# mdw771/beyond_dof

Hardware: AMD Instinct MI355X
Metric: multislice fwd+adjoint slice-steps/s (full Adam iteration: rotation, forward, loss, adjoint, gradient exchange, regulariser+Adam) (higher is better)
Workload: dtype f32

## Files before the change

### beyond_dof_amd/csrc/bdof_capi.hip

```cpp
#include <hip/hip_runtime.h>
#include <hip/hip_ext.h>
#include <cmath>
#include <algorithm>
#include <complex>
#include <cstdio>
#include <cstdlib>
#include <cstring>
#include <string>
#include <vector>

#include "../../include/bdof.h"
#include "bdof_steps.h"
#include "bdof_kernels.h"
#include "bdof_conv2.h"
#include "bdof_generic.h"
#include "bdof_field.h"
#include "bdof_conv64.h"
#include "bdof_resident.h"
#include "bdof_modes.h"
#include "bdof_comm.h"
#include "bdof_rigid.h"
#include "bdof_windows.h"
#include <rocfft/rocfft.h>
#include <map>
// ... 631 lines not shown
                    tw_of(c, c->twX, c->NX, tick)};
    sq_of(c, tick, a.sq);
    DISPATCH_N(c->NX, {
        if (gather) BDOF_LAUNCH(ps, (k_row_prop_gather<N_>), dim3(rows_grid<N_>(c, g.B, c->NY)), dim3(BDOF_THREADS), 0, g.st, a);
        else BDOF_LAUNCH(ps, (k_row_prop_fan<N_>), dim3(rows_grid<N_>(c, g.B, c->NY)), dim3(BDOF_THREADS), 0, g.st, a);
    });
}

static int fused_mode(const bdof_ctx* c) {
    if (c->fusion < 1 || c->sep_copies < 1 || c->recompute || c->bin != 1 || c->pstack || c->range_car) return 0;
    if (c->det_mode == BDOF_DET_FAR || c->obj.xoff || c->obj.yoff || c->gpsi0) return 0;
    if (c->S < 4 || (c->S & 1) || c->NX > 512 || c->NY > 512) return 0;
    return 1;
}
static LineSteps line_steps(bdof_ctx* c, bool x_lines, unsigned lead, unsigned trail) {
    const int N = x_lines ? c->NX : c->NY;
    const cf* tw = x_lines ? c->twX : c->twY;
    const cf* h = x_lines ? c->hx_d : c->hy_d;
    const unsigned D = (unsigned)c->sep_copies;
    LineSteps s{tw_of(c, tw, N, lead), tw_of(c, tw, N, trail), h + (size_t)(lead % D) * N, h + (size_t)(trail % D) * N};
    sq_of(c, lead, s.sq_lead);
    sq_of(c, trail, s.sq_trail);
    return s;
}
static void launch_slice(bdof_ctx* c, const Group& g, int z, const cf* in, cf* out, cf* phi, bool blk = false) {
    ProfScope ps(c, BDOF_K_ROW_FWD, g.st, true);
    const bool xl = (z & 1) != 0;
    const int N = xl ? c->NX : c->NY, R = xl ? c->NY : c->NX;
    SliceArgs a{sub_field(c, g, in), c->probe, sub_field(c, g, out), sub_field(c, g, phi), sub_obj(c, g), g.B, R, z, carrier_at(c, z), cshift_at(c, z),
                line_steps(c, xl, (unsigned)(z > 0 ? z - 1 : 0), (unsigned)z)};
    if (xl) {
        DISPATCH_N_512(N, with_bool(blk, [&](auto BLK) {
            BDOF_LAUNCH(ps, (k_slice_x<N_, BLK>), dim3(rows_grid<N_>(c, g.B, R)), dim3(BDOF_THREADS), 0, g.st, a);
        }));
    } else {
        DISPATCH_N_512(N, with_bool(z == 0, [&](auto FIRST) { with_bool(z == c->S - 2, [&](auto TAIL) {
            BDOF_LAUNCH(ps, (k_slice_y<N_, FIRST, TAIL>), dim3(rows_grid<N_>(c, g.B, R)), dim3(BDOF_THREADS), 0, g.st, a);
        }); }));
    }
}

static void launch_slice_adj(bdof_ctx* c, const Group& g, int z, const cf* in, cf* out, const cf* phi) {
    ProfScope ps(c, BDOF_K_ROW_BWD, g.st, true);
    const bool xl = (z & 1) != 0;
    const int N = xl ? c->NX : c->NY, R = xl ? c->NY : c->NX;
    SliceAdjArgs a{sub_field(c, g, in), sub_field(c, g, phi), sub_field(c, g, out), c->grot + (size_t)g.b0 * c->S * c->NX * c->NY, sub_obj(c, g), g.B, R, z,
                   c->k, carrier_phi_at(c, z), line_steps(c, xl, (unsigned)z, (unsigned)(z > 0 ? z - 1 : 0))};
    if (xl) {
        DISPATCH_N_512(N, BDOF_LAUNCH(ps, (k_slice_x_adj<N_>), dim3(rows_grid<N_>(c, g.B, R)), dim3(BDOF_THREADS), 0, g.st, a));
    } else {
        DISPATCH_N_512(N, with_bool(z == c->S - 2, [&](auto HEAD) { with_bool(z == 0, [&](auto LAST) {
            BDOF_LAUNCH(ps, (k_slice_y_adj<N_, HEAD, LAST>), dim3(rows_grid<N_>(c, g.B, R)), dim3(BDOF_THREADS), 0, g.st, a);
        }); }));
    }
}

struct GradTarget {
    float2* grot = nullptr;
    int S_ = 0, z_ = 0;
    cf* gpsi = nullptr;
};
static void launch_row_bwd(bdof_ctx* c, const Group& g, int z, const cf* gin, const cf* tape, cf* gout, int hist = 0, float tape_scale = 1.f,
                           const GradTarget* gt = nullptr) {
    ProfScope ps(c, BDOF_K_ROW_BWD, g.st, true);
    float2* grot = gt && gt->grot ? gt->grot + (size_t)g.b0 * gt->S_ * c->NX * c->NY : c->grot + (size_t)g.b0 * c->S * c->NX * c->NY;
    RowBwdArgs a{sub_field(c, g, gin), hist == 2 ? c->probe : sub_field(c, g, tape), sub_field(c, g, gout),
                 grot, sub_obj(c, g), g.B, c->NX, z, c->k, carrier_at(c, z), tw_of(c, c->twY, c->NY, (unsigned)z),
                 slice_carrier_field(c, z), adj_carrier_at(c, g, steps(c).steps_back(z)), cshift_at(c, z), carrier_phi_at(c, z), tape_scale,
                 gt && gt->gpsi ? sub_field(c, g, gt->gpsi) : (z == 0 ? sub_field<cf>(c, g, c->gpsi0) : nullptr),
                 gt && gt->grot ? gt->S_ : c->S, gt && gt->grot ? gt->z_ : steps(c).first_slice(z)};
    sq_of(c, (unsigned)z, a.sq);
    const int form = a.ac.gcar ? 2 : a.pz ? 1 : 0;
    if (c->bin > 1) {
        DISPATCH_N(c->NY, with_bool(hist == 2, [&](auto H2) { with_int<3>(form, [&](auto FORM) {
            BDOF_LAUNCH(ps, (k_row_bwd<N_, H2 ? 2 : 1, FORM == 1, FORM == 2, true>), dim3(rows_grid<N_>(c, g.B, c->NX)), dim3(BDOF_THREADS), 0, g.st, a);
        }); }));
        return;
    }
    DISPATCH_N(c->NY, with_int<4>(hist, [&](auto HIST) { with_int<3>(form, [&](auto FORM) {
        BDOF_LAUNCH(ps, (k_row_bwd<N_, HIST, FORM == 1, FORM == 2>), dim3(rows_grid<N_>(c, g.B, c->NX)), dim3(BDOF_THREADS), 0, g.st, a);
    }); }));
}

static LossArgs loss_args(bdof_ctx* c, const Group& g, const DetPlane& det, const cf* in, cf* out_hyb, cf* out_wave, const float* meas,
                          float in_scale, float out_scale, int part) {
    LossArgs a{};
    a.in = sub_field(c, g, in);
    a.out_hyb = sub_field(c, g, out_hyb);
    a.out_wave = sub_field(c, g, out_wave);
    a.meas = sub_field(c, g, meas);
    a.partial = c->partial + 2 * part;
    a.B = g.B;
    a.in_scale = in_scale;
    a.out_scale = out_scale;
    a.det = det;
    return a;
}
static int launch_loss_real(bdof_ctx* c, const Group& g, const DetPlane& det, const cf* in, cf* out_hyb, bool tstore, cf* out_wave, const float* meas,
                            float in_scale, float out_scale, int part = 0) {
    ProfScope ps(c, BDOF_K_LOSS, g.st);
    LossArgs a = loss_args(c, g, det, in, out_hyb, out_wave, meas, in_scale, out_scale, part);
    a.R = c->NX;
    a.twiddle = c->twY;
    int grid = 0;
    DISPATCH_N(c->NY, grid = rows_grid<N_>(c, g.B, c->NX); with_bool(tstore, [&](auto TSTORE) { with_bool(meas && loss_is_poisson(c), [&](auto PSN) {
        with_bool(meas && det.wgt, [&](auto WGT) { hipLaunchKernelGGL((k_row_loss<N_, false, TSTORE, PSN, WGT>), dim3(grid), dim3(BDOF_THREADS), 0, g.st, a); });
    }); }));
    return grid;
}

static int launch_loss_plane(bdof_ctx* c, const Group& g, const DetPlane& det, int j, cf* out_wave, const float* meas, int part = 0) {
    ProfScope ps(c, BDOF_K_LOSS, g.st);
    const size_t pl = (size_t)c->NX * c->NY;
    LossPlaneArgs a;
    static_cast<LossArgs&>(a) = loss_args(c, g, det, nullptr, nullptr, nullptr, nullptr, 1.f, 1.f, part);
    a.in = sub_planes<const cf>(c, g, c->det_pl) + j * pl;
    a.out_hyb = meas ? sub_planes<cf>(c, g, c->seed_pl) + j * pl : nullptr;
    a.out_wave = out_wave ? sub_planes(c, g, out_wave) + j * pl : nullptr;
    a.meas = meas ? sub_planes(c, g, meas) + j * pl : nullptr;
    a.fstride = c->planes;
    a.R = c->NX;
    a.twiddle = c->twY;
    int grid = 0;
    DISPATCH_N(c->NY, grid = rows_grid<N_>(c, g.B, c->NX); with_bool(meas && loss_is_poisson(c), [&](auto PSN) {
        with_bool(meas && det.wgt, [&](auto WGT) { hipLaunchKernelGGL((k_row_loss<N_, false, true, PSN, WGT, true>), dim3(grid), dim3(BDOF_THREADS), 0, g.st, a); });
    }));
    return grid;
}

static int launch_loss_far(bdof_ctx* c, const Group& g, const DetPlane& det, const cf* in, cf* out_hyb, cf* out_wave, const float* meas,
                           float in_scale, float out_scale, int part = 0) {
    ProfScope ps(c, BDOF_K_LOSS, g.st);
    LossArgs a = loss_args(c, g, det, in, out_hyb, out_wave, meas, in_scale, out_scale, part);
    a.R = c->NY;
    a.twiddle = c->twX;
    int grid = 0;
    DISPATCH_N(c->NX, grid = rows_grid<N_>(c, g.B, c->NY); with_bool(meas && loss_is_poisson(c), [&](auto PSN) {
        with_bool(meas && det.wgt, [&](auto WGT) { hipLaunchKernelGGL((k_row_loss<N_, true, true, PSN, WGT>), dim3(grid), dim3(BDOF_THREADS), 0, g.st, a); });
    }));
    return grid;
}

struct DetRoute {
    bool far;
    const cf* in;
    float in_scale;
    const cf* h;
    const cf* pfield;
};
static DetRoute det_route(const bdof_ctx* c) {
    const bool tf_all = c->variant == BDOF_VARIANT_TF_ALL;
    if (c->det_mode == BDOF_DET_FAR) return DetRoute{true, c->bufA, 1.f, nullptr, c->pdetT};
    if (c->det_mode == BDOF_DET_NONE && !tf_all) return DetRoute{false, c->bufA, 1.f / (float)c->NY, nullptr, c->pdet};
    return DetRoute{false, c->bufB, 1.f, c->det_mode == BDOF_DET_NONE ? c->hs : tf_all ? c->hcomb : c->hdet, c->pdet};
}

enum { TAPE_NONE = 0, TAPE_HISTORY = 1, TAPE_LAST = 2 };
static void forward_sweep(bdof_ctx* c, const Split& split, int tape_mode, bool fused = false, bool adj_fused = false) {
    const size_t fld = (size_t)c->Bmax * c->NX * c->NY;
    const DetRoute dr = det_route(c);
    const int nz = n_steps(c);
    for (int z = 0; z < nz; ++z) {
        const cf* in = nullptr;
        if (z > 0) in = tape_mode == TAPE_HISTORY ? c->tape + (size_t)steps(c).tape_read(z) * fld : c->bufB;
        const bool last = z == nz - 1;
        if (fused && last) in = c->tape + (size_t)z * fld;
        if (fused && !last) {
            for (const Group& g : split) {
                launch_slice(c, g, z, (z & 1) ? c->bufA : c->bufB, (z & 1) ? c->bufB : c->bufA, c->tape + (size_t)z * fld, adj_fused);
                if (z == nz - 2) launch_row_prop(c, g, c->bufA, c->tape + (size_t)(nz - 1) * fld, c->hx_rows, 1.f, 0, z, BDOF_K_LOSS);
            }
            continue;
        }
        cf* phi = tape_mode == TAPE_LAST && last ? c->tape : nullptr;
        for (const Group& g : split) {
            if (!last) {
                launch_row_fwd(c, g, z, in, c->bufA, true, phi);
                launch_row_prop(c, g, c->bufA, tape_mode == TAPE_HISTORY ? c->tape + (size_t)steps(c).tape_write(z) * fld : c->bufB, c->hs, 1.f, 0, z);
            } else {
                launch_row_fwd(c, g, z, in, c->bufA, dr.far || dr.h, phi);
                if (c->planes > 1) launch_row_planes(c, g, false, z, fused ? BDOF_K_LOSS : BDOF_K_COL_PROP);
                else if (dr.h) launch_row_prop(c, g, c->bufA, c->bufB, dr.h, 1.f, 0, z, fused ? BDOF_K_LOSS : BDOF_K_COL_PROP);
            }
        }
    }
}

static void march_back(bdof_ctx* c, const Group& g, int z, int hist, const cf* phi, bool phi_real, bool step, bool march, cf* rc1, cf* rc2,
                       const GradTarget* gt = nullptr) {
    launch_row_bwd(c, g, z, c->bufB, phi, step ? c->bufA : nullptr, hist, 1.f, gt);
    if (step) launch_row_prop(c, g, c->bufA, c->bufB, c->hs, 1.f, 1, z - 1);
    if (march) {
        launch_row_unmod(c, g, z, phi, rc2, phi_real, 1.f);
        launch_row_prop(c, g, rc2, rc1, c->hs, 1.f, 1, z - 1);
    }
}

static void adjoint_sweep(bdof_ctx* c, const Split& split, bool fused, bool adj_fused = false) {
    const size_t fld = (size_t)c->Bmax * c->NX * c->NY;
    const int nz = n_steps(c);
    for (int z = nz - 1; z >= 0; --z) {
        const bool top = z == nz - 1;
        for (const Group& g : split) {
            if (c->recompute) {
                march_back(c, g, z, z == 0 ? 2 : top ? 0 : 3, top ? c->tape : c->tape + fld, top, z > 0, z > 1, c->tape + fld, c->tape + 2 * fld);
                continue;
            }
            if (adj_fused && !top) {
                launch_slice_adj(c, g, z, (z & 1) ? c->bufA : c->bufB, (z & 1) ? c->bufB : c->bufA, c->tape + (size_t)z * fld);
                continue;
            }
            if (fused) launch_row_bwd(c, g, z, c->bufB, c->tape + (size_t)z * fld, z > 0 ? c->bufA : nullptr, top ? 1 : 0);
            else launch_row_bwd(c, g, z, c->bufB, z > 0 ? c->tape + (size_t)steps(c).tape_read(z) * fld : nullptr, z > 0 ? c->bufA : nullptr, z > 0 ? 1 : 2);
            if (z > 0) launch_row_prop(c, g, c->bufA, c->bufB, c->hs, 1.f, 1, z - 1);
        }
    }
}

static int modulation_room(bdof_ctx* c, size_t n, bool mean) {
    HIPC(c, c->mod.room(n));
// ... 1510 lines not shown
    if (!c || !probe || !hT) return BDOF_ERR_ARG;
    int r = enter_setter(c, true);
    if (r) return r;
    if (c->det_mode == BDOF_DET_NEAR && !hdetT) return fail(c, BDOF_ERR_ARG, "a near-field detector needs its transfer function in float64 too");
    const size_t n = (size_t)c->NX * c->NY;
    if ((r = upload(c, c->c64_probe, probe, n, KEEP)) || (r = upload(c, c->c64_h, hT, n, KEEP)) ||
        (hdetT && (r = upload(c, c->c64_hdet, hdetT, n, KEEP)))) return r;
    twin64_holds(c, true, 1);
    c->c64_k = k;
    return c64_room(c, c->Bmax, true, 0);
}

int bdof_loss_grad_tf_f64(bdof_ctx* c, int B, const int* angle_of_b, const int* xoff, const int* yoff, const float* meas, double meas_ref) {
    if (int r = admit(c, "bdof_loss_grad_tf_f64", NO_DATA_TERM)) return r;
    int r = ready_f64(c, B, angle_of_b, meas, c && c->c64_tf, "bdof_set_tf_f64 has not been called");
    if (r) return r;
    HIPC(c, hipSetDevice(c->device));
    if ((r = c64_room(c, B, true, 0))) return r;
    double2* psi = c->c64_psi;
    const Model64 m{c->c64_k, step_after_last(c),
                    [&](bool adj) { return free_step(c, c->fft, c->stream, psi, B, c->NX, c->NY, c->c64_h, H_KXKY, adj, true); }, nullptr};
    if ((r = sweep_f64(c, m, rows_view(c, angle_of_b, xoff, yoff), B, psi, c->c64_probe, 0, c->S, c->c64_tape, meas, meas_ref))) return r;
    return launched(c);
}

int bdof_tape_to_real(bdof_ctx* c, int i, int B, void* out) {
    int r = check_ready(c, B);
    if (r) return r;
    if (!out) return BDOF_ERR_ARG;
    if (!c->tape_valid) return fail(c, BDOF_ERR_STATE, "no history: run bdof_forward(keep_tape=1) first");
    const int nz = n_steps(c);
    if (i < 0 || i >= nz) return fail(c, BDOF_ERR_ARG, "slice index outside [0, S / slice binning)");
    const size_t fld = (size_t)c->Bmax * c->NX * c->NY;
    if (i < nz - 1) {
        launch_loss_real(c, whole(c, B), wave_plane(c, carrier_z(c, i + 1), slice_carrier_field(c, i + 1)), c->tape + (size_t)i * fld, nullptr, false,
                         (cf*)out, nullptr, 1.f, 1.f);
    } else {
        if (!c->last_valid)
            return fail(c, BDOF_ERR_STATE, "the last slice's wave is only kept after bdof_forward(keep_tape=1) with the numpy_skip_last variant");
        launch_loss_real(c, whole(c, B), wave_plane(c, carrier_z(c, nz - 1) * (1.0 + c->cbm1), slice_carrier_field(c, nz - 1)), c->bufA, nullptr, false,
                         (cf*)out, nullptr, 1.f / c->NY, 1.f);
    }
    return launched(c);
}

int bdof_loss_grad(bdof_ctx* c, int B, const int* angle_of_b, const int* xoff, const int* yoff, const float* meas, void* out_wave) {
    int r = check_ready(c, B);
    if (r) return r;
    if (!meas) return BDOF_ERR_ARG;
    if (c->meas_dev && (c->det_mode == BDOF_DET_FAR || c->pstack || c->n_modes))
        return fail(c, BDOF_ERR_STATE, "bdof_set_meas_mode(1) needs a real-space detector and a scalar carrier (not a carrier field, not probe modes)");
    if (!c->with_grad || !c->grot) return fail(c, BDOF_ERR_STATE, "bdof_loss_grad needs bdof_configure(with_grad=1) with the gradient workspace (not flag 32)");
    if ((r = need_angles(c, angle_of_b))) return r;
    if (c->n_modes && (r = check_modes_batch(c, B))) return r;
    if ((r = begin_batch(c, angle_of_b, xoff, yoff, c->k_fft))) return r;
    c->gpsi_src = c->gpsi0;
    c->gpsi_B = B;
    c->fused_last = c->adj_fused_last = 0;
    if (c->n_modes) {
        changed(c, TAPE_OVERWRITTEN);
        return modes_loss_grad(c, B, meas, out_wave);
    }
    if (use_resident(c, B)) {
        if ((r = resident_run(c, B, meas, out_wave, true))) return r;
        changed(c, TAPE_OVERWRITTEN);
        return 0;
    }
    if (c->generic) {
        if ((r = generic_loss_grad(c, B, meas, out_wave))) return r;
        changed(c, TAPE_OVERWRITTEN);
        c->gpsi_src = c->bufA;
        return launched(c);
    }
    Split split;
    if ((r = split.open(c, B, c->NX, 16))) return r;
    const bool fused = fused_mode(c) != 0;
    const bool adj_fused = fused && c->adj_fusion != 0;
    c->fused_last = fused ? 1 : 0;
    c->adj_fused_last = adj_fused ? 1 : 0;
    forward_sweep(c, split, c->recompute ? TAPE_LAST : TAPE_HISTORY, fused, adj_fused);
    changed(c, TAPE_OVERWRITTEN);
    int npart = 0;
    const DetRoute dr = det_route(c);
    for (const Group& g : split) {
        if (c->planes > 1) {
            for (int j = 0; j < c->planes; ++j)
                npart += launch_loss_plane(c, g, det_plane(c, g, B, nullptr, j), j, (cf*)out_wave, meas, npart);
            launch_row_planes(c, g, true, n_steps(c) - 1, fused ? BDOF_K_LOSS : BDOF_K_COL_PROP);
            continue;
        }
        const DetPlane det = det_plane(c, g, B, dr.pfield);
        if (dr.far) {
            npart += launch_loss_far(c, g, det, dr.in, c->bufB, (cf*)out_wave, meas, 1.f, 1.f, npart);
        } else if (!dr.h) {
            npart += launch_loss_real(c, g, det, dr.in, c->bufB, false, (cf*)out_wave, meas, dr.in_scale, dr.in_scale, npart);
        } else {
            npart += launch_loss_real(c, g, det, dr.in, c->bufA, true, (cf*)out_wave, meas, 1.f, 1.f, npart);
            launch_row_prop(c, g, c->bufA, c->bufB, dr.h, 1.f, 1, n_steps(c) - 1, fused ? BDOF_K_LOSS : BDOF_K_COL_PROP);
        }
    }
    adjoint_sweep(c, split, fused, adj_fused);
    if ((r = split.close(c))) return r;
    hipLaunchKernelGGL(k_sum_partials, dim3(1), dim3(256), 0, c->stream, c->partial, npart,
                       1.0 / ((double)B * c->planes * c->NX * c->NY), c->loss_dev);
    return launched(c);
}


int bdof_set_conv(bdof_ctx* c, const float* ky, const float* kx, int ks, double e_re, double e_im, double ksum_re,
                  double ksum_im, double k) {
    if (int r = admit(c, "bdof_set_conv", NO_DATA_TERM)) return r;
    if (!c || !ky || !kx) return BDOF_ERR_ARG;
    if (int r = enter_setter(c, false)) return r;
    if (ks < 1 || ks > BDOF_CONV_MAXK || ks % 2 == 0) return fail(c, BDOF_ERR_ARG, "kernel_size must be odd and <= 33");
    if (c->generic || c->NX % BDOF_CONV_TX || c->NY % BDOF_CONV_TY)
        return fail(c, BDOF_ERR_SIZE, "the conv propagator needs power-of-two wavefields (tiles are 32 x 64)");
    changed(c, CHANGED_CONV_TAPS);
    for (int i = 0; i < ks; ++i) {
        c->taps.ky[i] = make_float2(ky[2 * i], ky[2 * i + 1]);
        c->taps.kx[i] = make_float2(kx[2 * i], kx[2 * i + 1]);
    }
    c->taps.e = make_float2((float)e_re, (float)e_im);
    c->taps.ks = ks;
    c->ksum = std::complex<double>(ksum_re, ksum_im);
    c->k_conv = (float)k;
    const size_t fld = (size_t)c->Bmax * c->NX * c->NY;
    if (!c->bufC) HIPC(c, c->bufC.alloc(fld));
    if (!c->conv_scal) HIPC(c, c->conv_scal.alloc(4));
    HIPC(c, hipStreamSynchronize(c->stream));
    if (c->taps_copies != 1) c->taps_dev.reset();
    c->taps_copies = 1;
    if (int r = upload(c, c->taps_dev, &c->taps, 1, KEEP)) return r;
    c->have_conv = true;
    return 0;
}

int bdof_set_conv_taps_f64(bdof_ctx* c, const double* ky, const double* kx, double e_re, double e_im) {
    if (int r = admit(c, "bdof_set_conv_taps_f64", NO_DATA_TERM)) return r;
    if (!c || !ky || !kx) return BDOF_ERR_ARG;
    if (!c->have_conv) return fail(c, BDOF_ERR_STATE, "bdof_set_conv has not been called");
    const int D = c->tw_dither;
    if (D < 2) return 0;
    if (int r = enter_setter(c, false)) return r;
    std::vector<ConvTaps> t((size_t)D, c->taps);
    const int ks = c->taps.ks;
    for (int d = 0; d < D; ++d) {
        for (int i = 0; i < ks; ++i) {
            const double ph = 0.6180339887498949 * (4 * i + 1);
            t[d].ky[i] = make_float2(dither_pick(ky[2 * i], d, std::fmod(ph, 1.0)), dither_pick(ky[2 * i + 1], d, std::fmod(ph + 0.6180339887498949, 1.0)));
            t[d].kx[i] = make_float2(dither_pick(kx[2 * i], d, std::fmod(ph + 2 * 0.6180339887498949, 1.0)),
                                     dither_pick(kx[2 * i + 1], d, std::fmod(ph + 3 * 0.6180339887498949, 1.0)));
        }
        t[d].e = make_float2(dither_pick(e_re, d, 0.25), dither_pick(e_im, d, 0.75));
    }
    HIPC(c, hipStreamSynchronize(c->stream));
    if (int r = upload(c, c->taps_dev, t.data(), (size_t)D, FRESH)) return r;
    c->taps_copies = D;
    return 0;
}

}

static cf conv_carrier(const bdof_ctx* c, int z) {
    const std::complex<double> a = c->a0 * std::pow(c->ksum, z);
    return make_float2((float)a.real(), (float)a.imag());
}
static cf conv_pad(const bdof_ctx* c, int z) {
    const std::complex<double> a = (1.0 - c->a0) * std::pow(c->ksum, z);
    return make_float2((float)a.real(), (float)a.imag());
}

static int conv_lds_bytes(const bdof_ctx* c) {
    const int h = (c->taps.ks - 1) / 2;
    const int TXH = BDOF_CONV_TX + 2 * h, TYH = BDOF_CONV_TY + 2 * h;
    return (TXH * (TYH | 1) + TXH * (BDOF_CONV_TY + 1)) * (int)sizeof(cf);
}

static int conv_tiling() {
    const char* e = getenv("BDOF_CONV_TILING");
    return e && e[0] == '1' ? 1 : 2;
// ... 989 lines not shown
```

### beyond_dof_amd/csrc/bdof_kernels.h

```cpp
#pragma once
#include <type_traits>
#include "bdof_fft.h"

#define BDOF_THREADS 512

template <int N> struct RowCfg {
    static constexpr int T = N / 8;
    static constexpr int RPP = BDOF_THREADS / T;
    static constexpr int TILE = RPP > 16 ? RPP : 16;
    static constexpr int PASSES = TILE / RPP;
    static constexpr int NPAD = N + N / 16;
    static constexpr int RS = ((NPAD + 29) / 32) * 32 + 2;
    static constexpr int LDS_CF = TILE * RS;
    static constexpr int MIN_WAVES = N >= 1024 ? 2 : 4;
};

template <int T> struct RowLds {
    cf* base;
    __device__ __forceinline__ int slot(int i) const { return i + (i >> 4); }
    __device__ __forceinline__ cf ld_at(int base_slot, int c) const { return base[base_slot + c + (c >> 4)]; }
    __device__ __forceinline__ void st_at(int base_slot, int c, cf v) { base[base_slot + c + (c >> 4)] = v; }
    __device__ __forceinline__ void sync_w2r() { sync(); }
    __device__ __forceinline__ void sync_r2w() { sync(); }
    __device__ __forceinline__ void sync() {
// ... 746 lines not shown
                if constexpr (BIN) p[m] = gv;
                else gdst[tid + m * C::T] = gv;
                g[m] = cmulc(g[m], make_float2(1.f + db[m].x, db[m].y));
                if constexpr (GC) g[m] = cadd(g[m], cmulc(gam, csub(db[m], a.ac.cbm1)));
            }
            if constexpr (BIN) {
#pragma nounroll
                for (int j = 0; j < nbin; ++j, gdst += (size_t)a.NX * NY) {
#pragma unroll
                    for (int m = 0; m < 8; ++m) gdst[tid + m * C::T] = p[m];
                }
            }
            if (a.gpsi0) {
                cf* pd = a.gpsi0 + off;
#pragma unroll
                for (int m = 0; m < 8; ++m)
                    pd[tid + m * C::T] = GC ? cadd(g[m], cmulc(gam, make_float2(1.f + a.ac.cbm1.x, a.ac.cbm1.y))) : g[m];
            }
            if (a.gout) line_fft_partial<NY, -1, 1, EX>(g, tw, tid, lds);
        }
        if (a.gout) {
            __syncthreads();
            transposed_tail<NY, -1, 1, EX>(smem, a.gout + (size_t)b * NY * a.NX + x0, a.NX, 1.f, smem_tail, tw.sq);
            __syncthreads();
        }
    }
}

struct LineSteps {
    const cf* tw_lead;
    const cf* tw_trail;
    const cf* h_lead;
    const cf* h_trail;
    float sq_lead[2], sq_trail[2];
};

struct SliceArgs {
    const cf* in;
    const cf* probe;
    cf* out;
    cf* phi_out;
    ObjView obj;
    int B, R, z;
    cf carrier;
    cf cshift;
    LineSteps steps;
};
static_assert(offsetof(SliceArgs, steps) == 120 && sizeof(SliceArgs) == 168, "SliceArgs: the byte layout it had with the six members spelt out");

template <int N, int SIGN, int ROUND = 1>
__device__ __forceinline__ void transposed_tail_mul(cf* smem, cf* __restrict__ dst, size_t ld, const cf* __restrict__ h, const cf* tail, const float* sq) {
    typedef RowCfg<N> C;
#pragma nounroll
    for (int pass = 0; pass < C::PASSES; ++pass) {
        const auto [q, r, j] = transposed_at<C>(pass);
        RowLds<C::T> lds{smem + r * C::RS};
        cf u[8], hv[8];
#pragma unroll
        for (int m = 0; m < 8; ++m) hv[m] = h[j + m * C::T];
        last_stage<N, SIGN, ROUND, false>(u, j, lds, tail, sq);
#pragma unroll
        for (int m = 0; m < 8; ++m) dst[(size_t)(j + m * C::T) * ld + r] = cmul(u[m], hv[m]);
    }
}

struct ObjRows {
    const int* look;
    long long plain0;
    int imax;
    int xmax;
    int mask;
};
__device__ __forceinline__ ObjRows obj_rows_of(const ObjView o, int b, int z, int NX) {
    ObjRows r;
    r.look = o.tab ? o.tab + ((long long)o.angle_of_b[b] * o.S + z) * o.volNX : (const int*)o.vol;
    r.plain0 = o.tab ? 0 : ((long long)b * o.S + z) * NX;
    r.imax = o.tab ? o.volNX - 1 : 0;
    r.xmax = o.tab ? o.volNX - 1 : 0x7fffffff;
    r.mask = o.tab ? -1 : 0;
    return r;
}
__device__ __forceinline__ int obj_rows_rel(const ObjRows r, int x) {
    const int s = r.look[(unsigned)min(x, r.imax)] & r.mask;
    return x <= r.xmax ? s + (x & ~r.mask) : -1;
}

template <int N> __device__ __forceinline__ void tw_select(FftTw<N>& tw, const cf* mid, const cf* tail, const float* sq, int tid) {
    asm volatile("" ::: "memory");
    tw.mid = mid;
    tw.tail = tail;
    tw.sq = sq;
#pragma unroll
    for (int m = 1; m < 8; ++m) tw.w[m - 1] = tail[(m - 1) * (N / 8) + tid];
}

template <int NY, bool FIRST, bool TAIL>
__global__ __launch_bounds__(BDOF_THREADS, RowCfg<NY>::MIN_WAVES) void k_slice_y(SliceArgs a) {
    typedef RowCfg<NY> C;
    __shared__ cf smem[C::LDS_CF];
    __shared__ cf smem_tw[2][FftTw<NY>::LDS_CNT];
    __shared__ cf smem_tail[2][7 * C::T];
    const int tid = threadIdx.x % C::T, rl = threadIdx.x / C::T;
    const float sql[2] = {a.steps.sq_lead[0], a.steps.sq_lead[1]}, sqt[2] = {a.steps.sq_trail[0], a.steps.sq_trail[1]};
    FftTw<NY> tw;
    if constexpr (!FIRST) FftTw<NY>::fill(a.steps.tw_lead, smem_tw[0], smem_tail[0]);
    FftTw<NY>::fill(a.steps.tw_trail, smem_tw[1], smem_tail[1]);
    __syncthreads();
    const int NX = a.R;
    const int ntiles = a.B * NX / C::TILE;
    for (int tile = blockIdx.x; tile < ntiles; tile += gridDim.x) {
        const auto [row0, b, x0] = tile_at<C>(tile, NX);
#pragma nounroll
        for (int pass = 0; pass < C::PASSES; ++pass) {
            const int r = pass * C::RPP + rl;
            const int x = x0 + r;
            RowLds<C::T> lds{smem + r * C::RS};
            cf u[8], hv[8];
            float2 db[8];
            const cf* src = FIRST ? a.probe + (size_t)x * NY : a.in + (size_t)(row0 + r) * NY;
#pragma unroll
            for (int m = 0; m < 8; ++m) u[m] = src[tid + m * C::T];
            load_obj_row(a.obj, obj_src_row(a.obj, b, x, a.z, NX), 0, tid, C::T, db);
            if constexpr (!FIRST) {
#pragma unroll
                for (int m = 0; m < 8; ++m) hv[m] = a.steps.h_lead[tid + m * C::T];
                tw_select(tw, smem_tw[0], smem_tail[0], sql, tid);
                line_fft<NY, -1, 1, false>(u, tw, tid, lds);
#pragma unroll
                for (int m = 0; m < 8; ++m) u[m] = cmul(u[m], hv[m]);
                line_fft<NY, +1, 2, false>(u, tw, tid, lds);
            }
#pragma unroll
            for (int m = 0; m < 8; ++m) u[m] = modulate_eps_s(u[m], a.carrier, db[m], a.cshift);
            cf* pdst = a.phi_out + (size_t)(row0 + r) * NY;
#pragma unroll
            for (int m = 0; m < 8; ++m) pdst[tid + m * C::T] = u[m];
            tw_select(tw, smem_tw[1], smem_tail[1], sqt, tid);
            if constexpr (TAIL) {
                line_fft_partial<NY, -1, 1, false>(u, tw, tid, lds);
            } else {
#pragma unroll
                for (int m = 0; m < 8; ++m) hv[m] = a.steps.h_trail[tid + m * C::T];
                line_fft<NY, -1, 1, false>(u, tw, tid, lds);
#pragma unroll
                for (int m = 0; m < 8; ++m) u[m] = cmul(u[m], hv[m]);
                line_fft_partial<NY, +1, 2, false>(u, tw, tid, lds);
            }
        }
        __syncthreads();
        cf* dst = a.out + (size_t)b * NY * NX + x0;
        if constexpr (TAIL) transposed_tail_mul<NY, -1, 1>(smem, dst, NX, a.steps.h_trail, smem_tail[1], sqt);
        else transposed_tail<NY, +1, 2, false>(smem, dst, NX, 1.f, smem_tail[1], sqt);
        __syncthreads();
    }
}

template <int NX, bool BLK = false>
__global__ __launch_bounds__(BDOF_THREADS, RowCfg<NX>::MIN_WAVES) void k_slice_x(SliceArgs a) {
    typedef RowCfg<NX> C;
    typedef FftPlan<NX> P;
    __shared__ cf smem[C::LDS_CF];
    __shared__ cf smem_tw[2][FftTw<NX>::LDS_CNT];
    __shared__ cf smem_tail[2][7 * C::T];
    const int tid = threadIdx.x % C::T, rl = threadIdx.x / C::T;
    const float sql[2] = {a.steps.sq_lead[0], a.steps.sq_lead[1]}, sqt[2] = {a.steps.sq_trail[0], a.steps.sq_trail[1]};
    __shared__ int s_src[NX];
    FftTw<NX> tw;
    FftTw<NX>::fill(a.steps.tw_lead, smem_tw[0], smem_tail[0]);
    FftTw<NX>::fill(a.steps.tw_trail, smem_tw[1], smem_tail[1]);
    __syncthreads();
    const ObjView o = a.obj;
    const int NY = a.R;
    const int ntiles = a.B * NY / C::TILE;
    for (int tile = blockIdx.x; tile < ntiles; tile += gridDim.x) {
        const auto [row0, b, y0] = tile_at<C>(tile, NY);
        const ObjRows rows = obj_rows_of(o, b, a.z, NX);
        cf* const pdst = a.phi_out + (BLK ? (size_t)row0 * NX : (size_t)b * NX * NY);
        const int src_mine = (int)threadIdx.x < NX ? obj_rows_rel(rows, threadIdx.x) : -1;
#pragma nounroll
        for (int pass = 0; pass < C::PASSES; ++pass) {
            const int r = pass * C::RPP + rl;
            RowLds<C::T> lds{smem + r * C::RS};
            cf u[8], hv[8];
            const cf* src = a.in + (size_t)(row0 + r) * NX;
#pragma unroll
            for (int m = 0; m < 8; ++m) u[m] = src[tid + m * C::T];
#pragma unroll
            for (int m = 0; m < 8; ++m) hv[m] = a.steps.h_lead[tid + m * C::T];
            tw_select(tw, smem_tw[0], smem_tail[0], sql, tid);
            line_fft<NX, -1, 1, false>(u, tw, tid, lds);
#pragma unroll
            for (int m = 0; m < 8; ++m) u[m] = cmul(u[m], hv[m]);
            line_fft_partial<NX, +1, 2, false>(u, tw, tid, lds);
        }
        if ((int)threadIdx.x < NX) s_src[threadIdx.x] = src_mine;
        __syncthreads();
        cf v[C::PASSES][8];
#pragma unroll
        for (int pass = 0; pass < C::PASSES; ++pass) {
            const auto [q, r, j] = transposed_at<C>(pass);
            RowLds<C::T> lds{smem + r * C::RS};
            const int yg = y0 + r, yc = min(max(yg, 0), o.volNY - 1);
            float2 db[8];
#pragma unroll
            for (int m = 0; m < 8; ++m) {
                const int srel = s_src[j + m * C::T];
                const float2 t = o.vol[(size_t)(rows.plain0 + max(srel, 0)) * o.volNY + yc];
                const bool in = srel >= 0 && yg == yc;
                db[m] = make_float2(in ? t.x : 0.f, in ? t.y : 0.f);
            }
            last_stage<NX, +1, 2, false>(v[pass], j, lds, smem_tail[0], sql);
#pragma unroll
            for (int m = 0; m < 8; ++m) {
                v[pass][m] = modulate_eps_s(v[pass][m], a.carrier, db[m], a.cshift);
                if constexpr (BLK) pdst[(unsigned)(q + m * C::T * C::TILE)] = v[pass][m];
                else pdst[(unsigned)((j + m * C::T) * NY + yg)] = v[pass][m];
            }
            tw.sq = sqt;
            stage_compute<NX, -1, P::R0, 1, 0, 1, false>(v[pass], tw, j);
        }
        __syncthreads();
#pragma unroll
        for (int pass = 0; pass < C::PASSES; ++pass) {
            const auto [q, r, j] = transposed_at<C>(pass);
            RowLds<C::T> lds{smem + r * C::RS};
            stage_write<NX, P::R0, 1>(v[pass], j, lds);
        }
        __syncthreads();
#pragma nounroll
        for (int pass = 0; pass < C::PASSES; ++pass) {
            const int r = pass * C::RPP + rl;
            RowLds<C::T> lds{smem + r * C::RS};
            cf u[8], hv[8];
#pragma unroll
            for (int m = 0; m < 8; ++m) hv[m] = a.steps.h_trail[tid + m * C::T];
            tw_select(tw, smem_tw[1], smem_tail[1], sqt, tid);
            line_fft_rest<NX, -1, 1, false>(u, tw, tid, lds);
#pragma unroll
            for (int m = 0; m < 8; ++m) u[m] = cmul(u[m], hv[m]);
            line_fft_partial<NX, +1, 2, false>(u, tw, tid, lds);
        }
        __syncthreads();
        transposed_tail<NX, +1, 2, false>(smem, a.out + (size_t)b * NX * NY + y0, NY, 1.f, smem_tail[1], sqt);
        __syncthreads();
    }
}

struct SliceAdjArgs {
    const cf* in;
    const cf* phi;
    cf* out;
    float2* grot;
    ObjView obj;
    int B, R, z;
    float k;
    cf carrier_phi;
    LineSteps steps;
};
static_assert(offsetof(SliceAdjArgs, steps) == 112 && sizeof(SliceAdjArgs) == 160, "SliceAdjArgs: the byte layout it had with the six members spelt out");

template <int NY, bool HEAD, bool LAST>
__global__ __launch_bounds__(BDOF_THREADS, RowCfg<NY>::MIN_WAVES) void k_slice_y_adj(SliceAdjArgs a) {
    typedef RowCfg<NY> C;
    __shared__ cf smem[C::LDS_CF];
    __shared__ cf smem_tw[2][FftTw<NY>::LDS_CNT];
    __shared__ cf smem_tail[2][7 * C::T];
    const int tid = threadIdx.x % C::T, rl = threadIdx.x / C::T;
    const float sql[2] = {a.steps.sq_lead[0], a.steps.sq_lead[1]}, sqt[2] = {a.steps.sq_trail[0], a.steps.sq_trail[1]};
    FftTw<NY> tw;
    FftTw<NY>::fill(a.steps.tw_lead, smem_tw[0], smem_tail[0]);
    if constexpr (!LAST) FftTw<NY>::fill(a.steps.tw_trail, smem_tw[1], smem_tail[1]);
    __syncthreads();
    const int NX = a.R;
    const int ntiles = a.B * NX / C::TILE;
    for (int tile = blockIdx.x; tile < ntiles; tile += gridDim.x) {
        const auto [row0, b, x0] = tile_at<C>(tile, NX);
#pragma nounroll
        for (int pass = 0; pass < C::PASSES; ++pass) {
            const int r = pass * C::RPP + rl;
            const int x = x0 + r;
            RowLds<C::T> lds{smem + r * C::RS};
            const size_t off = (size_t)(row0 + r) * NY;
            cf g[8], p[8], hv[8];
            float2 db[8];
#pragma unroll
            for (int m = 0; m < 8; ++m) g[m] = a.in[off + tid + m * C::T];
            if constexpr (!HEAD) {
#pragma unroll
                for (int m = 0; m < 8; ++m) hv[m] = a.steps.h_lead[tid + m * C::T];
            }
            auto load_phi_and_table = [&, b = b]() {
#pragma unroll
                for (int m = 0; m < 8; ++m) p[m] = a.phi[off + tid + m * C::T];
                load_obj_row(a.obj, obj_src_row(a.obj, b, x, a.z, NX), 0, tid, C::T, db);
            };
            tw_select(tw, smem_tw[0], smem_tail[0], sql, tid);
            if constexpr (HEAD) {
                load_phi_and_table();
                line_fft<NY, +1, 1, false>(g, tw, tid, lds);
            } else {
                line_fft<NY, -1, 1, false>(g, tw, tid, lds);
#pragma unroll
                for (int m = 0; m < 8; ++m) g[m] = cmulc(g[m], hv[m]);
                load_phi_and_table();
                line_fft<NY, +1, 2, false>(g, tw, tid, lds);
            }
            float2* gdst = a.grot + (((size_t)b * a.obj.S + a.z) * NX + x) * NY;
#pragma unroll
            for (int m = 0; m < 8; ++m) {
                const cf t = cmulc(g[m], cadd(p[m], a.carrier_phi));
                gdst[tid + m * C::T] = make_float2(a.k * t.y, -a.k * t.x);
                g[m] = cmulc(g[m], make_float2(1.f + db[m].x, db[m].y));
            }
            if constexpr (!LAST) {
#pragma unroll
                for (int m = 0; m < 8; ++m) hv[m] = a.steps.h_trail[tid + m * C::T];
                tw_select(tw, smem_tw[1], smem_tail[1], sqt, tid);
                line_fft<NY, -1, 1, false>(g, tw, tid, lds);
#pragma unroll
                for (int m = 0; m < 8; ++m) g[m] = cmulc(g[m], hv[m]);
                line_fft_partial<NY, +1, 2, false>(g, tw, tid, lds);
            }
        }
        if constexpr (!LAST) {
            __syncthreads();
            transposed_tail<NY, +1, 2, false>(smem, a.out + (size_t)b * NY * NX + x0, NX, 1.f, smem_tail[1], sqt);
            __syncthreads();
        }
    }
}

template <int NX>
__global__ __launch_bounds__(BDOF_THREADS, RowCfg<NX>::MIN_WAVES) void k_slice_x_adj(SliceAdjArgs a) {
    typedef RowCfg<NX> C;
    typedef FftPlan<NX> P;
    __shared__ cf smem[C::LDS_CF];
    __shared__ cf smem_tw[2][FftTw<NX>::LDS_CNT];
    __shared__ cf smem_tail[2][7 * C::T];
    const int tid = threadIdx.x % C::T, rl = threadIdx.x / C::T;
    const float sql[2] = {a.steps.sq_lead[0], a.steps.sq_lead[1]}, sqt[2] = {a.steps.sq_trail[0], a.steps.sq_trail[1]};
    __shared__ int s_src[NX];
    FftTw<NX> tw;
    FftTw<NX>::fill(a.steps.tw_lead, smem_tw[0], smem_tail[0]);
    FftTw<NX>::fill(a.steps.tw_trail, smem_tw[1], smem_tail[1]);
    __syncthreads();
    const ObjView o = a.obj;
    const int NY = a.R;
    const int ntiles = a.B * NY / C::TILE;
    for (int tile = blockIdx.x; tile < ntiles; tile += gridDim.x) {
        const auto [row0, b, y0] = tile_at<C>(tile, NY);
        const ObjRows rows = obj_rows_of(o, b, a.z, NX);
        const cf* const psrc = a.phi + (size_t)row0 * NX;
        float2* const gdst = a.grot + ((size_t)b * o.S + a.z) * NX * NY;
        const int src_mine = (int)threadIdx.x < NX ? obj_rows_rel(rows, threadIdx.x) : -1;
#pragma nounroll
        for (int pass = 0; pass < C::PASSES; ++pass) {
            const int r = pass * C::RPP + rl;
            RowLds<C::T> lds{smem + r * C::RS};
            cf u[8], hv[8];
            const cf* src = a.in + (size_t)(row0 + r) * NX;
#pragma unroll
            for (int m = 0; m < 8; ++m) u[m] = src[tid + m * C::T];
#pragma unroll
            for (int m = 0; m < 8; ++m) hv[m] = a.steps.h_lead[tid + m * C::T];
            tw_select(tw, smem_tw[0], smem_tail[0], sql, tid);
            line_fft<NX, -1, 1, false>(u, tw, tid, lds);
#pragma unroll
            for (int m = 0; m < 8; ++m) u[m] = cmulc(u[m], hv[m]);
            line_fft_partial<NX, +1, 2, false>(u, tw, tid, lds);
        }
        if ((int)threadIdx.x < NX) s_src[threadIdx.x] = src_mine;
        __syncthreads();
        cf v[C::PASSES][8];
#pragma unroll
        for (int pass = 0; pass < C::PASSES; ++pass) {
            const auto [q, r, j] = transposed_at<C>(pass);
            RowLds<C::T> lds{smem + r * C::RS};
            const int yg = y0 + r, yc = min(max(yg, 0), o.volNY - 1);
            float2 db[8];
            cf p[8];
#pragma unroll
            for (int m = 0; m < 8; ++m) {
                const int srel = s_src[j + m * C::T];
                const float2 t = o.vol[(size_t)(rows.plain0 + max(srel, 0)) * o.volNY + yc];
                const bool in = srel >= 0 && yg == yc;
                db[m] = make_float2(in ? t.x : 0.f, in ? t.y : 0.f);
            }
#pragma unroll
            for (int m = 0; m < 8; ++m) p[m] = psrc[(unsigned)(q + m * C::T * C::TILE)];
            last_stage<NX, +1, 2, false>(v[pass], j, lds, smem_tail[0], sql);
#pragma unroll
            for (int m = 0; m < 8; ++m) {
                const cf t = cmulc(v[pass][m], cadd(p[m], a.carrier_phi));
                gdst[(unsigned)((j + m * C::T) * NY + yg)] = make_float2(a.k * t.y, -a.k * t.x);
                v[pass][m] = cmulc(v[pass][m], make_float2(1.f + db[m].x, db[m].y));
            }
            tw.sq = sqt;
            stage_compute<NX, -1, P::R0, 1, 0, 1, false>(v[pass], tw, j);
        }
        __syncthreads();
#pragma unroll
        for (int pass = 0; pass < C::PASSES; ++pass) {
            const auto [q, r, j] = transposed_at<C>(pass);
            RowLds<C::T> lds{smem + r * C::RS};
            stage_write<NX, P::R0, 1>(v[pass], j, lds);
        }
        __syncthreads();
#pragma nounroll
        for (int pass = 0; pass < C::PASSES; ++pass) {
            const int r = pass * C::RPP + rl;
            RowLds<C::T> lds{smem + r * C::RS};
            cf u[8], hv[8];
#pragma unroll
            for (int m = 0; m < 8; ++m) hv[m] = a.steps.h_trail[tid + m * C::T];
            tw_select(tw, smem_tw[1], smem_tail[1], sqt, tid);
            line_fft_rest<NX, -1, 1, false>(u, tw, tid, lds);
#pragma unroll
            for (int m = 0; m < 8; ++m) u[m] = cmulc(u[m], hv[m]);
            line_fft_partial<NX, +1, 2, false>(u, tw, tid, lds);
        }
        __syncthreads();
        transposed_tail<NX, +1, 2, false>(smem, a.out + (size_t)b * NX * NY + y0, NY, 1.f, smem_tail[1], sqt);
        __syncthreads();
    }
}

struct AdamArgs {
    const float2* x_old;
    float2* x_new;
    const float2* g;
    float2* m;
    float2* v;
    const float* mask;
    int NXv, NZv, NYv;
    float g_scale;
    float alpha_d, alpha_b, gamma;
    float lr, b1, b2, eps, inv_bc1, inv_bc2;
    float om_b1, om_b2;
    int clip;
    int x0, x1;
};

__device__ __forceinline__ float sgn(float v) { return (v > 0.f) - (v < 0.f); }

template <bool STORE_MV, class G>
__device__ __forceinline__ void adam_voxel(const AdamArgs& a, size_t idx, int x, int z, int y, G grad, float& nd, float& nb, float2& m, float2& v) {
    const float2 xv = a.x_old[idx];
    const float2 g = grad();
    float gd = g.x * a.g_scale + a.alpha_d * sgn(xv.x);
    float gb = g.y * a.g_scale + a.alpha_b * sgn(xv.y);
    if (a.gamma != 0.f) {
        const size_t sy = 1, sz = a.NYv, sx = (size_t)a.NZv * a.NYv;
        const float ym = a.x_old[idx - y * sy + ((y + a.NYv - 1) % a.NYv) * sy].x;
        const float yp = a.x_old[idx - y * sy + ((y + 1) % a.NYv) * sy].x;
        const float zm = a.x_old[idx - z * sz + ((z + a.NZv - 1) % a.NZv) * sz].x;
        const float zp = a.x_old[idx - z * sz + ((z + 1) % a.NZv) * sz].x;
        const float xm = a.x_old[idx - x * sx + ((x + a.NXv - 1) % a.NXv) * sx].x;
        const float xp = a.x_old[idx - x * sx + ((x + 1) % a.NXv) * sx].x;
        const float c = xv.x;
        gd += a.gamma * (sgn(c - ym) - sgn(yp - c) + sgn(c - zm) - sgn(zp - c) + sgn(c - xm) - sgn(xp - c));
    }
    m = a.m[idx];
    v = a.v[idx];
    m.x = a.om_b1 * gd + a.b1 * m.x;
    m.y = a.om_b1 * gb + a.b1 * m.y;
    v.x = a.om_b2 * gd * gd + a.b2 * v.x;
    v.y = a.om_b2 * gb * gb + a.b2 * v.y;
    if constexpr (STORE_MV) {
        a.m[idx] = m;
        a.v[idx] = v;
    }
    nd = xv.x - a.lr * (m.x * a.inv_bc1) / (sqrtf(v.x * a.inv_bc2) + a.eps);
    nb = xv.y - a.lr * (m.y * a.inv_bc1) / (sqrtf(v.y * a.inv_bc2) + a.eps);
    if (a.mask) { const float mk = a.mask[idx]; nd *= mk; nb *= mk; }
    if (a.clip) { nd = fmaxf(nd, 0.f); nb = fmaxf(nb, 0.f); }
}

struct RotAdjArgs {
    const float2* grot;
    float2* gvol;
    const int* off;
    const int* order;
    const int* angle_of_b;
    int B, n_src, n_dest, NY, accumulate;
    float scale;
    int* heavy_count;
// ... 903 lines not shown
```

Measured before the change: 234,700.

## Prefetch object table via wave shuffles and size loss grid per tile

In the slice forward and backward kernels, the shared-memory source-row table is replaced by per-lane lookups that are broadcast with wave shuffles. Object-volume and phi loads are issued early and software-pipelined across passes, with asm barriers pinning where they are scheduled, so the FFT stages hide their latency. Separately, the loss kernels launch one block per tile when the tile count fits the partial-sum buffer. The cost is higher register pressure from holding several prefetched passes, and the kernels now rely on wave-size assumptions enforced by static_asserts.

```diff
diff --git a/beyond_dof_amd/csrc/bdof_capi.hip b/beyond_dof_amd/csrc/bdof_capi.hip
--- a/beyond_dof_amd/csrc/bdof_capi.hip
+++ b/beyond_dof_amd/csrc/bdof_capi.hip
@@ -737,6 +737,16 @@
     }); }));
 }
 
+template <int N> static int loss_grid(const bdof_ctx* c, int B, int R, bool per_tile) {
+    return per_tile ? B * R / RowCfg<N>::TILE : rows_grid<N>(c, B, R);
+}
+static bool loss_tiles_fit(const bdof_ctx* c, int B, bool far) {
+    if (c->planes > 1) return false;
+    long long tiles = 0;
+    DISPATCH_N(far ? c->NX : c->NY, tiles = (long long)B * (far ? c->NY : c->NX) / RowCfg<N_>::TILE);
+    return tiles > 0 && tiles <= c->npartial;
+}
+
 static LossArgs loss_args(bdof_ctx* c, const Group& g, const DetPlane& det, const cf* in, cf* out_hyb, cf* out_wave, const float* meas,
                           float in_scale, float out_scale, int part) {
     LossArgs a{};
@@ -752,13 +762,13 @@
     return a;
 }
 static int launch_loss_real(bdof_ctx* c, const Group& g, const DetPlane& det, const cf* in, cf* out_hyb, bool tstore, cf* out_wave, const float* meas,
-                            float in_scale, float out_scale, int part = 0) {
+                            float in_scale, float out_scale, int part = 0, bool per_tile = false) {
     ProfScope ps(c, BDOF_K_LOSS, g.st);
     LossArgs a = loss_args(c, g, det, in, out_hyb, out_wave, meas, in_scale, out_scale, part);
     a.R = c->NX;
     a.twiddle = c->twY;
     int grid = 0;
-    DISPATCH_N(c->NY, grid = rows_grid<N_>(c, g.B, c->NX); with_bool(tstore, [&](auto TSTORE) { with_bool(meas && loss_is_poisson(c), [&](auto PSN) {
+    DISPATCH_N(c->NY, grid = loss_grid<N_>(c, g.B, c->NX, per_tile); with_bool(tstore, [&](auto TSTORE) { with_bool(meas && loss_is_poisson(c), [&](auto PSN) {
         with_bool(meas && det.wgt, [&](auto WGT) { hipLaunchKernelGGL((k_row_loss<N_, false, TSTORE, PSN, WGT>), dim3(grid), dim3(BDOF_THREADS), 0, g.st, a); });
     }); }));
     return grid;
@@ -784,13 +794,13 @@
 }
 
 static int launch_loss_far(bdof_ctx* c, const Group& g, const DetPlane& det, const cf* in, cf* out_hyb, cf* out_wave, const float* meas,
-                           float in_scale, float out_scale, int part = 0) {
+                           float in_scale, float out_scale, int part = 0, bool per_tile = false) {
     ProfScope ps(c, BDOF_K_LOSS, g.st);
     LossArgs a = loss_args(c, g, det, in, out_hyb, out_wave, meas, in_scale, out_scale, part);
     a.R = c->NY;
     a.twiddle = c->twX;
     int grid = 0;
-    DISPATCH_N(c->NX, grid = rows_grid<N_>(c, g.B, c->NY); with_bool(meas && loss_is_poisson(c), [&](auto PSN) {
+    DISPATCH_N(c->NX, grid = loss_grid<N_>(c, g.B, c->NY, per_tile); with_bool(meas && loss_is_poisson(c), [&](auto PSN) {
         with_bool(meas && det.wgt, [&](auto WGT) { hipLaunchKernelGGL((k_row_loss<N_, true, true, PSN, WGT>), dim3(grid), dim3(BDOF_THREADS), 0, g.st, a); });
     }));
     return grid;
@@ -2467,6 +2477,7 @@
     changed(c, TAPE_OVERWRITTEN);
     int npart = 0;
     const DetRoute dr = det_route(c);
+    const bool per_tile = loss_tiles_fit(c, B, dr.far);
     for (const Group& g : split) {
         if (c->planes > 1) {
             for (int j = 0; j < c->planes; ++j)
@@ -2476,11 +2487,11 @@
         }
         const DetPlane det = det_plane(c, g, B, dr.pfield);
         if (dr.far) {
-            npart += launch_loss_far(c, g, det, dr.in, c->bufB, (cf*)out_wave, meas, 1.f, 1.f, npart);
+            npart += launch_loss_far(c, g, det, dr.in, c->bufB, (cf*)out_wave, meas, 1.f, 1.f, npart, per_tile);
         } else if (!dr.h) {
-            npart += launch_loss_real(c, g, det, dr.in, c->bufB, false, (cf*)out_wave, meas, dr.in_scale, dr.in_scale, npart);
+            npart += launch_loss_real(c, g, det, dr.in, c->bufB, false, (cf*)out_wave, meas, dr.in_scale, dr.in_scale, npart, per_tile);
         } else {
-            npart += launch_loss_real(c, g, det, dr.in, c->bufA, true, (cf*)out_wave, meas, 1.f, 1.f, npart);
+            npart += launch_loss_real(c, g, det, dr.in, c->bufA, true, (cf*)out_wave, meas, 1.f, 1.f, npart, per_tile);
             launch_row_prop(c, g, c->bufA, c->bufB, dr.h, 1.f, 1, n_steps(c) - 1, fused ? BDOF_K_LOSS : BDOF_K_COL_PROP);
         }
     }
diff --git a/beyond_dof_amd/csrc/bdof_kernels.h b/beyond_dof_amd/csrc/bdof_kernels.h
--- a/beyond_dof_amd/csrc/bdof_kernels.h
+++ b/beyond_dof_amd/csrc/bdof_kernels.h
@@ -852,7 +852,13 @@
 }
 __device__ __forceinline__ int obj_rows_rel(const ObjRows r, int x) {
     const int s = r.look[(unsigned)min(x, r.imax)] & r.mask;
-    return x <= r.xmax ? s + (x & ~r.mask) : -1;
+    const int none = -(int)(x > r.xmax);
+    return ((s + (x & ~r.mask)) & ~none) | none;
+}
+
+__device__ __forceinline__ void use_from_here(float2 (&v)[8]) {
+#pragma unroll
+    for (int m = 0; m < 8; ++m) asm volatile("" : "+v"(v[m].x), "+v"(v[m].y));
 }
 
 template <int N> __device__ __forceinline__ void tw_select(FftTw<N>& tw, const cf* mid, const cf* tail, const float* sq, int tid) {
@@ -925,6 +931,21 @@
     }
 }
 
+template <class C> struct WaveRows {
+    static_assert(C::TILE <= 64 && 64 % C::TILE == 0 && BDOF_THREADS % 64 == 0, "a wave covers whole values of j");
+    static constexpr int JW = 64 / C::TILE;
+    static constexpr int JP = BDOF_THREADS / C::TILE;
+    static_assert(JW * C::PASSES * 8 <= 64, "one lookup per lane");
+    static __device__ __forceinline__ int x_mine() {
+        const int lane = threadIdx.x % 64, w = threadIdx.x / 64;
+        const int i = lane % JW, t = lane / JW;
+        return w * JW + i + (t % C::PASSES) * JP + (t / C::PASSES) * C::T;
+    }
+    static __device__ __forceinline__ int get(int mine, int pass, int m) {
+        return __shfl(mine, (int)(threadIdx.x % 64) / C::TILE + JW * (pass + C::PASSES * m), 64);
+    }
+};
+
 template <int NX, bool BLK = false>
 __global__ __launch_bounds__(BDOF_THREADS, RowCfg<NX>::MIN_WAVES) void k_slice_x(SliceArgs a) {
     typedef RowCfg<NX> C;
@@ -934,20 +955,33 @@
     __shared__ cf smem_tail[2][7 * C::T];
     const int tid = threadIdx.x % C::T, rl = threadIdx.x / C::T;
     const float sql[2] = {a.steps.sq_lead[0], a.steps.sq_lead[1]}, sqt[2] = {a.steps.sq_trail[0], a.steps.sq_trail[1]};
-    __shared__ int s_src[NX];
+    typedef WaveRows<C> W;
     FftTw<NX> tw;
     FftTw<NX>::fill(a.steps.tw_lead, smem_tw[0], smem_tail[0]);
     FftTw<NX>::fill(a.steps.tw_trail, smem_tw[1], smem_tail[1]);
     __syncthreads();
     const ObjView o = a.obj;
+    const float2* const __restrict__ vol = o.vol;
     const int NY = a.R;
     const int ntiles = a.B * NY / C::TILE;
     for (int tile = blockIdx.x; tile < ntiles; tile += gridDim.x) {
         const auto [row0, b, y0] = tile_at<C>(tile, NY);
         const ObjRows rows = obj_rows_of(o, b, a.z, NX);
-        cf* const pdst = a.phi_out + (BLK ? (size_t)row0 * NX : (size_t)b * NX * NY);
-        const int src_mine = (int)threadIdx.x < NX ? obj_rows_rel(rows, threadIdx.x) : -1;
-#pragma nounroll
+        cf* const __restrict__ pdst = a.phi_out + (BLK ? (size_t)row0 * NX : (size_t)b * NX * NY);
+        const int src_mine = obj_rows_rel(rows, W::x_mine());
+        const int yg = y0 + (int)(threadIdx.x % C::TILE), yc = min(max(yg, 0), o.volNY - 1);
+        float2 db[C::PASSES][8];
+        unsigned inb[C::PASSES];
+        auto request_table = [&](int pass) {
+            inb[pass] = 0;
+#pragma unroll
+            for (int m = 0; m < 8; ++m) {
+                const int srel = W::get(src_mine, pass, m);
+                db[pass][m] = vol[(size_t)(rows.plain0 + max(srel, 0)) * o.volNY + yc];
+                inb[pass] |= (unsigned)(srel >= 0 && yg == yc) << m;
+            }
+        };
+#pragma unroll
         for (int pass = 0; pass < C::PASSES; ++pass) {
             const int r = pass * C::RPP + rl;
             RowLds<C::T> lds{smem + r * C::RS};
@@ -961,28 +995,23 @@
             line_fft<NX, -1, 1, false>(u, tw, tid, lds);
 #pragma unroll
             for (int m = 0; m < 8; ++m) u[m] = cmul(u[m], hv[m]);
+            if (pass == C::PASSES - 1) request_table(0);
             line_fft_partial<NX, +1, 2, false>(u, tw, tid, lds);
         }
-        if ((int)threadIdx.x < NX) s_src[threadIdx.x] = src_mine;
         __syncthreads();
         cf v[C::PASSES][8];
+#pragma unroll
+        for (int pass = 1; pass < C::PASSES; ++pass) request_table(pass);
 #pragma unroll
         for (int pass = 0; pass < C::PASSES; ++pass) {
             const auto [q, r, j] = transposed_at<C>(pass);
             RowLds<C::T> lds{smem + r * C::RS};
-            const int yg = y0 + r, yc = min(max(yg, 0), o.volNY - 1);
-            float2 db[8];
+            last_stage<NX, +1, 2, false>(v[pass], j, lds, smem_tail[0], sql);
+            use_from_here(db[pass]);
 #pragma unroll
             for (int m = 0; m < 8; ++m) {
-                const int srel = s_src[j + m * C::T];
-                const float2 t = o.vol[(size_t)(rows.plain0 + max(srel, 0)) * o.volNY + yc];
-                const bool in = srel >= 0 && yg == yc;
-                db[m] = make_float2(in ? t.x : 0.f, in ? t.y : 0.f);
-            }
-            last_stage<NX, +1, 2, false>(v[pass], j, lds, smem_tail[0], sql);
-#pragma unroll
-            for (int m = 0; m < 8; ++m) {
-                v[pass][m] = modulate_eps_s(v[pass][m], a.carrier, db[m], a.cshift);
+                const bool in = inb[pass] >> m & 1;
+                v[pass][m] = modulate_eps_s(v[pass][m], a.carrier, make_float2(in ? db[pass][m].x : 0.f, in ? db[pass][m].y : 0.f), a.cshift);
                 if constexpr (BLK) pdst[(unsigned)(q + m * C::T * C::TILE)] = v[pass][m];
                 else pdst[(unsigned)((j + m * C::T) * NY + yg)] = v[pass][m];
             }
@@ -1107,23 +1136,38 @@
     __shared__ cf smem[C::LDS_CF];
     __shared__ cf smem_tw[2][FftTw<NX>::LDS_CNT];
     __shared__ cf smem_tail[2][7 * C::T];
-    const int tid = threadIdx.x % C::T, rl = threadIdx.x / C::T;
     const float sql[2] = {a.steps.sq_lead[0], a.steps.sq_lead[1]}, sqt[2] = {a.steps.sq_trail[0], a.steps.sq_trail[1]};
-    __shared__ int s_src[NX];
+    typedef WaveRows<C> W;
     FftTw<NX> tw;
     FftTw<NX>::fill(a.steps.tw_lead, smem_tw[0], smem_tail[0]);
     FftTw<NX>::fill(a.steps.tw_trail, smem_tw[1], smem_tail[1]);
     __syncthreads();
     const ObjView o = a.obj;
+    const float2* const __restrict__ vol = o.vol;
     const int NY = a.R;
     const int ntiles = a.B * NY / C::TILE;
     for (int tile = blockIdx.x; tile < ntiles; tile += gridDim.x) {
         const auto [row0, b, y0] = tile_at<C>(tile, NY);
+        int tx = threadIdx.x;
+        if constexpr (C::PASSES > 1) asm volatile("" : "+v"(tx));
+        const int tid = tx % C::T, rl = tx / C::T;
         const ObjRows rows = obj_rows_of(o, b, a.z, NX);
-        const cf* const psrc = a.phi + (size_t)row0 * NX;
-        float2* const gdst = a.grot + ((size_t)b * o.S + a.z) * NX * NY;
-        const int src_mine = (int)threadIdx.x < NX ? obj_rows_rel(rows, threadIdx.x) : -1;
-#pragma nounroll
+        const cf* const __restrict__ psrc = a.phi + (size_t)row0 * NX;
+        float2* const __restrict__ gdst = a.grot + ((size_t)b * o.S + a.z) * NX * NY;
+        const int src_mine = obj_rows_rel(rows, W::x_mine());
+        const int yg = y0 + tx % C::TILE, yc = min(max(yg, 0), o.volNY - 1);
+        float2 db[C::PASSES][8];
+        unsigned inb[C::PASSES];
+        auto request_table = [&](int pass) {
+            inb[pass] = 0;
+#pragma unroll
+            for (int m = 0; m < 8; ++m) {
+                const int srel = W::get(src_mine, pass, m);
+                db[pass][m] = vol[(size_t)(rows.plain0 + max(srel, 0)) * o.volNY + yc];
+                inb[pass] |= (unsigned)(srel >= 0 && yg == yc) << m;
+            }
+        };
+#pragma unroll
         for (int pass = 0; pass < C::PASSES; ++pass) {
             const int r = pass * C::RPP + rl;
             RowLds<C::T> lds{smem + r * C::RS};
@@ -1137,41 +1181,46 @@
             line_fft<NX, -1, 1, false>(u, tw, tid, lds);
 #pragma unroll
             for (int m = 0; m < 8; ++m) u[m] = cmulc(u[m], hv[m]);
+            if (pass == C::PASSES - 1) request_table(0);
             line_fft_partial<NX, +1, 2, false>(u, tw, tid, lds);
         }
-        if ((int)threadIdx.x < NX) s_src[threadIdx.x] = src_mine;
         __syncthreads();
         cf v[C::PASSES][8];
+        cf p[C::PASSES][8];
+        auto request_phi = [&](int pass) {
+#pragma unroll
+            for (int m = 0; m < 8; ++m) p[pass][m] = psrc[(unsigned)(tx + pass * BDOF_THREADS + m * C::T * C::TILE)];
+        };
+        request_phi(0);
 #pragma unroll
         for (int pass = 0; pass < C::PASSES; ++pass) {
-            const auto [q, r, j] = transposed_at<C>(pass);
+            const int q = tx + pass * BDOF_THREADS, r = q % C::TILE, j = q / C::TILE;
             RowLds<C::T> lds{smem + r * C::RS};
-            const int yg = y0 + r, yc = min(max(yg, 0), o.volNY - 1);
-            float2 db[8];
-            cf p[8];
+            last_stage<NX, +1, 2, false>(v[pass], j, lds, smem_tail[0], sql);
+            if (pass + 1 < C::PASSES) request_table(pass + 1);
+            use_from_here(p[pass]);
+            use_from_here(db[pass]);
+            float2 gv[8];
 #pragma unroll
             for (int m = 0; m < 8; ++m) {
-                const int srel = s_src[j + m * C::T];
-                const float2 t = o.vol[(size_t)(rows.plain0 + max(srel, 0)) * o.volNY + yc];
-                const bool in = srel >= 0 && yg == yc;
-                db[m] = make_float2(in ? t.x : 0.f, in ? t.y : 0.f);
-            }
-#pragma unroll
-            for (int m = 0; m < 8; ++m) p[m] = psrc[(unsigned)(q + m * C::T * C::TILE)];
-            last_stage<NX, +1, 2, false>(v[pass], j, lds, smem_tail[0], sql);
-#pragma unroll
-            for (int m = 0; m < 8; ++m) {
-                const cf t = cmulc(v[pass][m], cadd(p[m], a.carrier_phi));
-                gdst[(unsigned)((j + m * C::T) * NY + yg)] = make_float2(a.k * t.y, -a.k * t.x);
-                v[pass][m] = cmulc(v[pass][m], make_float2(1.f + db[m].x, db[m].y));
-            }
+                const bool in = inb[pass] >> m & 1;
+                const cf t = cmulc(v[pass][m], cadd(p[pass][m], a.carrier_phi));
+                gv[m] = make_float2(a.k * t.y, -a.k * t.x);
+                v[pass][m] = cmulc(v[pass][m], make_float2(1.f + (in ? db[pass][m].x : 0.f), in ? db[pass][m].y : 0.f));
+            }
+            if (pass + 1 < C::PASSES) {
+                asm volatile("" ::: "memory");
+                request_phi(pass + 1);
+            }
+#pragma unroll
+            for (int m = 0; m < 8; ++m) gdst[(unsigned)((j + m * C::T) * NY + yg)] = gv[m];
             tw.sq = sqt;
             stage_compute<NX, -1, P::R0, 1, 0, 1, false>(v[pass], tw, j);
         }
         __syncthreads();
 #pragma unroll
         for (int pass = 0; pass < C::PASSES; ++pass) {
-            const auto [q, r, j] = transposed_at<C>(pass);
+            const int q = tx + pass * BDOF_THREADS, r = q % C::TILE, j = q / C::TILE;
             RowLds<C::T> lds{smem + r * C::RS};
             stage_write<NX, P::R0, 1>(v[pass], j, lds);
         }
```

Result: faster. 241,600 (median of 6 runs) (+2.9%).
